# dfdazac/grapes

Hardware: AMD Instinct MI355X
Metric: sampled edges aggregated/sec, ogbn-products 3-layer GFlowNet (higher is better)
Workload: dtype f32

## Files before the change

### grapes_amd/csrc/index_kernels.hip

```cpp
#include "common.h"

__global__ void tensormap_update_k(int32_t* __restrict__ map, const int32_t* __restrict__ keys,
                                   int n_host, const int32_t* d_n) {
    const int n = eff_count(d_n, n_host);
    for (int i = blockIdx.x * blockDim.x + threadIdx.x; i < n; i += gridDim.x * blockDim.x)
        map[keys[i]] = i;
}

__global__ void tensormap_map_k(const int32_t* __restrict__ map, const int32_t* __restrict__ keys,
                                int32_t* __restrict__ out, int64_t n_host, const int32_t* d_n) {
    int64_t n = n_host;
    if (d_n) { int64_t v = *d_n; n = v < n_host ? v : n_host; }
    for (int64_t i = (int64_t)blockIdx.x * blockDim.x + threadIdx.x; i < n;
         i += (int64_t)gridDim.x * blockDim.x)
        out[i] = map[keys[i]];
}

extern "C" int grapes_tensormap_update(int32_t* map, const int32_t* keys, int32_t n,
                                       const int32_t* d_n, grapes_stream_t stream) {
    if (!map || (!keys && n > 0) || n < 0) return GRAPES_EINVAL;
    if (n == 0) return 0;
    int grid = grapes_div_up(n, 256); if (grid > 2048) grid = 2048;
    hipLaunchKernelGGL(tensormap_update_k, dim3(grid), dim3(256), 0, (hipStream_t)stream, map, keys, n, d_n);
    GRAPES_LAUNCH_CHECK();
// ... 473 lines not shown
    int grid = grapes_div_up(n, 256); if (grid > 4096) grid = 4096;
    hipLaunchKernelGGL(bitmap_mark_k, dim3(grid), dim3(256), 0, (hipStream_t)stream,
                       (unsigned long long*)bits, (unsigned long long*)bits1, ids, n, d_n, num_nodes, status);
    GRAPES_LAUNCH_CHECK();
    return 0;
}

__global__ void bitmap_mark_rows_k(unsigned long long* __restrict__ bits, unsigned long long* __restrict__ bits1,
                                   const int32_t* __restrict__ nodes, int m_host, const int32_t* d_m,
                                   const int32_t* __restrict__ eoff, int num_nodes, int32_t* status) {
    const int m = eff_count(d_m, m_host);
    for (int i = blockIdx.x * blockDim.x + threadIdx.x; i < m; i += gridDim.x * blockDim.x) {
        if (eoff[i + 1] <= eoff[i]) continue;
        const int id = nodes[i];
        if (id < 0 || id >= num_nodes) {
            if (status) atomicOr(status, GRAPES_STATUS_BAD_INDEX);
            continue;
        }
        const int w = id >> 6;
        const unsigned long long old = atomicOr(&bits[w], 1ull << (id & 63));
        if (bits1 && old == 0ull) atomicOr(&bits1[w >> 6], 1ull << (w & 63));
    }
}

extern "C" int grapes_bitmap_mark_rows(uint64_t* bits, uint64_t* bits1, const int32_t* nodes, int32_t m,
                                       const int32_t* d_m, const int32_t* eoff, int32_t num_nodes, int32_t* status,
                                       grapes_stream_t stream) {
    if (!bits || m < 0 || (m > 0 && (!nodes || !eoff))) return GRAPES_EINVAL;
    if (m == 0) return 0;
    int grid = grapes_div_up(m, 256); if (grid > 1024) grid = 1024;
    hipLaunchKernelGGL(bitmap_mark_rows_k, dim3(grid), dim3(256), 0, (hipStream_t)stream, (unsigned long long*)bits,
                       (unsigned long long*)bits1, nodes, m, d_m, eoff, num_nodes, status);
    GRAPES_LAUNCH_CHECK();
    return 0;
}

__global__ void bitmap_mark_hop_k(unsigned long long* __restrict__ prev_bits, unsigned long long* __restrict__ bits,
                                  unsigned long long* __restrict__ bits1, const int32_t* __restrict__ previous,
                                  int m_host, const int32_t* d_m, const int32_t* __restrict__ eoff,
                                  const int32_t* __restrict__ dst, int e_host, const int32_t* d_e, int num_nodes,
                                  int32_t* status) {
    const int m = eff_count(d_m, m_host);
    const int e = eff_count(d_e, e_host);
    const int stride = gridDim.x * blockDim.x;
    const int i0 = blockIdx.x * blockDim.x + threadIdx.x;
    for (int i = i0; i < m; i += stride) {
        const int id = previous[i];
        mark_bit(prev_bits, nullptr, id, num_nodes, status);
        if (eoff[i + 1] > eoff[i]) mark_bit(bits, bits1, id, num_nodes, status);
    }
    for (int t = i0; t < e; t += stride) mark_bit(bits, bits1, dst[t], num_nodes, status);
}

extern "C" int grapes_bitmap_mark_hop(uint64_t* prev_bits, uint64_t* bits, uint64_t* bits1, const int32_t* previous,
                                      int32_t m, const int32_t* d_m, const int32_t* eoff, const int32_t* dst, int32_t e,
                                      const int32_t* d_e, int32_t num_nodes, int32_t* status, grapes_stream_t stream) {
    if (!prev_bits || !bits || m < 0 || e < 0 || (m > 0 && (!previous || !eoff)) || (e > 0 && !dst))
        return GRAPES_EINVAL;
    if (m == 0 && e == 0) return 0;
    int grid = grapes_div_up(m > e ? m : e, 256); if (grid > 4096) grid = 4096;
    hipLaunchKernelGGL(bitmap_mark_hop_k, dim3(grid), dim3(256), 0, (hipStream_t)stream, (unsigned long long*)prev_bits,
                       (unsigned long long*)bits, (unsigned long long*)bits1, previous, m, d_m, eoff, dst, e, d_e, num_nodes,
                       status);
    GRAPES_LAUNCH_CHECK();
    return 0;
}

struct MarkLists { const int32_t* ids[4]; int n[4]; const int32_t* d_n[4]; };
__global__ void bitmap_mark_lists_k(unsigned long long* __restrict__ bits, unsigned long long* __restrict__ bits1,
                                    MarkLists L, int num_nodes, int32_t* status, int32_t* __restrict__ unmark_mult) {
    const int stride = gridDim.x * blockDim.x;
    const int i0 = blockIdx.x * blockDim.x + threadIdx.x;
#pragma unroll
    for (int k = 0; k < 4; ++k) {
        if (!L.ids[k]) continue;
        const int n = eff_count(L.d_n[k], L.n[k]);
        for (int i = i0; i < n; i += stride) {
            const int id = L.ids[k][i];
            mark_bit(bits, bits1, id, num_nodes, status);
            if (unmark_mult && id >= 0 && id < num_nodes) unmark_mult[id] = 0;
        }
    }
}

extern "C" int grapes_bitmap_mark_lists(uint64_t* bits, uint64_t* bits1, const int32_t* ids0, int32_t n0,
                                        const int32_t* d_n0, const int32_t* ids1, int32_t n1, const int32_t* d_n1,
                                        const int32_t* ids2, int32_t n2, const int32_t* d_n2, const int32_t* ids3,
                                        int32_t n3, const int32_t* d_n3, int32_t num_nodes, int32_t* status,
                                        int32_t* unmark_mult, grapes_stream_t stream) {
    if (!bits || n0 < 0 || n1 < 0 || n2 < 0 || n3 < 0) return GRAPES_EINVAL;
    MarkLists L{{n0 > 0 ? ids0 : nullptr, n1 > 0 ? ids1 : nullptr, n2 > 0 ? ids2 : nullptr, n3 > 0 ? ids3 : nullptr},
                {n0, n1, n2, n3}, {d_n0, d_n1, d_n2, d_n3}};
    int nmax = n0; if (n1 > nmax) nmax = n1; if (n2 > nmax) nmax = n2; if (n3 > nmax) nmax = n3;
    if (nmax == 0) return 0;
    int grid = grapes_div_up(nmax, 256); if (grid > 4096) grid = 4096;
    hipLaunchKernelGGL(bitmap_mark_lists_k, dim3(grid), dim3(256), 0, (hipStream_t)stream, (unsigned long long*)bits,
                       (unsigned long long*)bits1, L, num_nodes, status, unmark_mult);
    GRAPES_LAUNCH_CHECK();
    return 0;
}

#define UNION_MAX 4096
template <int KPT>
__device__ __forceinline__ void union_sort_regs(int* key, int tid, int P) {
    int v[KPT];
#pragma unroll
    for (int q = 0; q < KPT; ++q) v[q] = key[tid + 1024 * q];
    for (int k = 2; k <= P; k <<= 1)
        for (int j = k >> 1; j > 0; j >>= 1) {
            if (j >= 1024) {
                const int dq = j >> 10;
#pragma unroll
                for (int q = 0; q < KPT; ++q) {
                    if ((q & dq) == 0 && (q | dq) < KPT) {
                        const int q2 = q | dq;
                        const bool up = ((tid + 1024 * q) & k) == 0;
                        const int a = v[q], b = v[q2];
                        const int mn = a < b ? a : b, mx = a < b ? b : a;
                        v[q] = up ? mn : mx; v[q2] = up ? mx : mn;
                    }
                }
                continue;
            }
            int partner[KPT];
            if (j >= 64) {
                __syncthreads();
#pragma unroll
                for (int q = 0; q < KPT; ++q) key[tid + 1024 * q] = v[q];
                __syncthreads();
#pragma unroll
                for (int q = 0; q < KPT; ++q) partner[q] = key[(tid + 1024 * q) ^ j];
            } else {
#pragma unroll
                for (int q = 0; q < KPT; ++q) partner[q] = __shfl_xor(v[q], j, 64);
            }
#pragma unroll
            for (int q = 0; q < KPT; ++q) {
                const int i = tid + 1024 * q;
                const bool up = (i & k) == 0, lower = (i & j) == 0;
                const int mn = v[q] < partner[q] ? v[q] : partner[q], mx = v[q] < partner[q] ? partner[q] : v[q];
                v[q] = (lower == up) ? mn : mx;
            }
        }
    __syncthreads();
#pragma unroll
    for (int q = 0; q < KPT; ++q) key[tid + 1024 * q] = v[q];
    __syncthreads();
}
__device__ __forceinline__ void union_sorted_body(MarkLists L, int num_nodes, int n_cap, int32_t* __restrict__ out_ids,
                                                       int32_t* __restrict__ node_map, int32_t* __restrict__ counts,
                                                       int32_t* __restrict__ unmark_mult, int32_t* status) {
    __shared__ int key[UNION_MAX];
    __shared__ int lds[17];
    __shared__ int s_total;
    const int tid = threadIdx.x;
    int nh[4], cv[4], id0[4];
#pragma unroll
    for (int k = 0; k < 4; ++k) {
        nh[k] = L.ids[k] ? L.n[k] : 0;
        const int32_t* pc = (L.ids[k] && L.d_n[k]) ? L.d_n[k] : counts;
        cv[k] = *pc;
    }
#pragma unroll
    for (int k = 0; k < 4; ++k) {
        const int32_t* pi = L.ids[k] ? L.ids[k] : counts;
        id0[k] = pi[(L.ids[k] && tid < nh[k]) ? tid : 0];
    }
    int off = 0;
    bool bad = false;
#pragma unroll
    for (int k = 0; k < 4; ++k) {
        if (!L.ids[k]) continue;
        int n = nh[k];
        if (L.d_n[k]) { n = cv[k] < nh[k] ? (cv[k] < 0 ? 0 : cv[k]) : nh[k]; }
        for (int i = tid; i < n; i += blockDim.x) {
            const int id = i == tid ? id0[k] : L.ids[k][i];
            const bool ok = id >= 0 && id < num_nodes;
            bad = bad || !ok;
            key[off + i] = ok ? id : 0x7fffffff;
        }
        off += n;
    }
    int P = 1; while (P < off) P <<= 1;
    for (int i = off + tid; i < P; i += blockDim.x) key[i] = 0x7fffffff;
    if (bad && status) atomicOr(status, GRAPES_STATUS_BAD_INDEX);
    __syncthreads();
    if (P <= (int)blockDim.x) {
        int v = tid < P ? key[tid] : 0x7fffffff;
        for (int k = 2; k <= P; k <<= 1)
            for (int j = k >> 1; j > 0; j >>= 1) {
                int partner;
                if (j >= 64) {
                    __syncthreads();
                    key[tid] = v;
                    __syncthreads();
                    partner = key[tid ^ j];
                } else {
                    partner = __shfl_xor(v, j, 64);
                }
                const bool up = (tid & k) == 0, lower = (tid & j) == 0;
                const int mn = v < partner ? v : partner, mx = v < partner ? partner : v;
                v = (lower == up) ? mn : mx;
            }
        __syncthreads();
        key[tid] = v;
        __syncthreads();
    } else if (blockDim.x == 1024 && (P == 2048 || P == 4096)) {
        if (P == 2048) union_sort_regs<2>(key, tid, P); else union_sort_regs<4>(key, tid, P);
    } else
    for (int k = 2; k <= P; k <<= 1)
        for (int j = k >> 1; j > 0; j >>= 1) {
            for (int i = tid; i < P; i += blockDim.x) {
                const int ixj = i ^ j;
                if (ixj > i) {
                    const int a = key[i], b = key[ixj];
                    const bool up = (i & k) == 0;
                    if ((a > b) == up) { key[i] = b; key[ixj] = a; }
                }
            }
            __syncthreads();
        }
    const int per = (P + (int)blockDim.x - 1) / (int)blockDim.x;
    const int lo = tid * per, hi = lo + per < P ? lo + per : P;
    int mine = 0;
    for (int i = lo; i < hi; ++i) { const int v = key[i]; if (v != 0x7fffffff && (i == 0 || key[i - 1] != v)) ++mine; }
    int tot;
    int pos = block_excl_scan(mine, lds, &tot);
    bool overflow = false;
    for (int i = lo; i < hi; ++i) {
        const int v = key[i];
        if (v != 0x7fffffff && (i == 0 || key[i - 1] != v)) {
            if (pos < n_cap) { out_ids[pos] = v; if (node_map) node_map[v] = pos; }
            else overflow = true;
            if (unmark_mult) unmark_mult[v] = 0;
            ++pos;
        }
    }
    if (tid == 0) { counts[0] = tot < n_cap ? tot : n_cap; counts[1] = counts[0]; }
    if (overflow && status) atomicOr(status, GRAPES_STATUS_NODE_OVERFLOW);
    (void)s_total;
}

__global__ __launch_bounds__(1024) void union_sorted_k(MarkLists L, int num_nodes, int n_cap, int32_t* __restrict__ out_ids,
                                                       int32_t* __restrict__ node_map, int32_t* __restrict__ counts,
                                                       int32_t* __restrict__ unmark_mult, int32_t* status) {
    union_sorted_body(L, num_nodes, n_cap, out_ids, node_map, counts, unmark_mult, status);
}

extern "C" int grapes_bitmap_clear(uint64_t* bits, const int32_t* ids, int64_t n, const int32_t* d_n,
                                   grapes_stream_t stream) {
    if (!bits || (!ids && n > 0) || n < 0) return GRAPES_EINVAL;
    if (n == 0) return 0;
    int grid = grapes_div_up(n, 256); if (grid > 4096) grid = 4096;
    hipLaunchKernelGGL(bitmap_clear_k, dim3(grid), dim3(256), 0, (hipStream_t)stream,
                       (unsigned long long*)bits, ids, n, d_n);
    GRAPES_LAUNCH_CHECK();
    return 0;
}

__global__ __launch_bounds__(1024) void compact_count_k(const unsigned long long* __restrict__ bits,
                                                        const unsigned long long* __restrict__ prev_bits, int W,
                                                        int32_t* __restrict__ bsum_b, int32_t* __restrict__ bsum_n) {
    __shared__ int lds[17];
    const int q = blockIdx.x * blockDim.x + threadIdx.x;
    int cb = 0, cn = 0;
    if (q < W) {
        const unsigned long long bb = bits[q];
        if (bb) {
            const unsigned long long pp = prev_bits ? prev_bits[q] : 0ull;
            cb = __popcll(bb); cn = __popcll(bb & ~pp);
        }
    }
    int tb, tn;
    block_excl_scan(cb, lds, &tb);
    block_excl_scan(cn, lds, &tn);
    if (threadIdx.x == 0) { bsum_b[blockIdx.x] = tb; bsum_n[blockIdx.x] = tn; }
}

__device__ __forceinline__ void long_row_items(const grapes_hop_degree_args& hd, int row, int ct, int cs) {
    if (ct > GRAPES_LONG_ROW) {
        const int nc = (ct + GRAPES_LONG_ROW - 1) / GRAPES_LONG_ROW;
        const int b0 = atomicAdd(&hd.n_long[0], nc);
        for (int c = 0; c < nc; ++c)
            if (b0 + c < hd.item_cap) { hd.long_items[2 * (b0 + c)] = row; hd.long_items[2 * (b0 + c) + 1] = c; }
    }
    if (cs > GRAPES_LONG_ROW) {
        const int nc = (cs + GRAPES_LONG_ROW - 1) / GRAPES_LONG_ROW;
        const int b0 = atomicAdd(&hd.n_long[1], nc);
        for (int c = 0; c < nc; ++c)
            if (b0 + c < hd.item_cap) { hd.long_items[2 * (hd.item_cap + b0 + c)] = row; hd.long_items[2 * (hd.item_cap + b0 + c) + 1] = c; }
    }
}

__device__ __forceinline__ void compact_emit_body(unsigned long long* __restrict__ bits,
                                                       const unsigned long long* __restrict__ prev_bits, int W,
                                                       const int32_t* __restrict__ bsum_b, const int32_t* __restrict__ bsum_n,
                                                       int n_cap, int32_t* __restrict__ batch_nodes,
                                                       int32_t* __restrict__ neighbor_nodes, int32_t* __restrict__ nb_local,
                                                       int32_t* __restrict__ node_map, int32_t* __restrict__ counts,
                                                       int32_t* status, uint32_t* __restrict__ ind_code,
                                                       uint32_t epoch_host, const uint32_t* d_epoch, int ind_bit,
                                                       unsigned long long* __restrict__ sync, int32_t* __restrict__ cand_pos,
                                                       uint32_t* __restrict__ zero_a, size_t words_a,
                                                       uint32_t* __restrict__ zero_b, size_t words_b,
                                                       uint32_t* __restrict__ zero_c, size_t words_c,
                                                       grapes_slice_remark_args rm, int gc,
                                                       grapes_hop_degree_args hd, const int BID, const int NBLK) {
    const int sj_t = blockDim.x > 64 ? (int)blockDim.x - 64 : (int)blockDim.x, sj_0 = blockDim.x > 64 ? (int)threadIdx.x - 64 : (int)threadIdx.x;
    if (BID >= gc) {
        if (sj_0 < 0) return;
        const size_t stride = (size_t)NBLK * sj_t, i0 = (size_t)BID * sj_t + sj_0;
        if (rm.mult) {
            if (rm.unmark_ids) { const int c = eff_count(rm.d_n_unmark, rm.n_unmark); for (size_t i = i0; i < (size_t)c; i += stride) rm.mult[rm.unmark_ids[i]] = 0; }
            if (rm.mark_ids) { const int c = eff_count(rm.d_n_mark, rm.n_mark); for (size_t i = i0; i < (size_t)c; i += stride) atomicAdd(&rm.mult[rm.mark_ids[i]], 1); }
        }
        for (size_t i = i0; i < words_a; i += stride) zero_a[i] = 0u;
        for (size_t i = i0; i < words_b; i += stride) zero_b[i] = 0u;
        for (size_t i = i0; i < words_c; i += stride) zero_c[i] = 0u;
        return;
    }
    __shared__ int lds[51];
    __shared__ unsigned long long lds64[2];
    GRAPES_STAMP_NW(0);
    const uint32_t epoch = d_epoch ? (*d_epoch & 0xffffffu) : epoch_host;
    const int w = BID * blockDim.x + threadIdx.x;
    unsigned long long bb = 0ull, pp = 0ull;
    int wt = 0, wsv = 0;
    if (w < W) {
        bb = bits[w];
        pp = prev_bits ? prev_bits[w] : 0ull;
        if (hd.indeg) { wt = hd.wsum[w]; wsv = hd.wsum[W + w]; }
    }
    GRAPES_STAMP(1);
    int tb, tn;
    int posb, posn;
    int post = 0, poss = 0, tt = 0, ts = 0;
    if (blockDim.x <= 512 && hd.indeg) {
        int pk = __popcll(bb) | (__popcll(bb & ~pp) << 16), tot;
        post = wt; poss = wsv;
        block_excl_scan3(pk, post, poss, lds, &tot, &tt, &ts);
        posb = pk & 0xffff; posn = (int)((unsigned)pk >> 16); tb = tot & 0xffff; tn = (int)((unsigned)tot >> 16);
    } else if (blockDim.x <= 512) {
        int tot;
        const int pk = block_excl_scan(__popcll(bb) | (__popcll(bb & ~pp) << 16), lds, &tot);
        posb = pk & 0xffff; posn = (int)((unsigned)pk >> 16); tb = tot & 0xffff; tn = (int)((unsigned)tot >> 16);
    } else {
        posb = block_excl_scan(__popcll(bb), lds, &tb);
        posn = block_excl_scan(__popcll(bb & ~pp), lds, &tn);
    }
    GRAPES_STAMP_NW(7);
    if (sync && threadIdx.x == 0)
        __hip_atomic_store(&sync[1 + BID], (1ull << 63) | ((unsigned long long)tn << 31) | (unsigned)tb, __ATOMIC_RELAXED, __HIP_MEMORY_SCOPE_AGENT);
    constexpr int PRE = 4;
    int l_ct[PRE] = {0, 0, 0, 0}, l_lp[PRE] = {0, 0, 0, 0};
    uint32_t l_cd[PRE] = {0u, 0u, 0u, 0u};
    int2 l_sg[PRE] = {make_int2(0, 0), make_int2(0, 0), make_int2(0, 0), make_int2(0, 0)};
    if (hd.indeg) {
        if (blockDim.x > 512) {
            post = block_excl_scan(wt, lds, &tt);
            poss = block_excl_scan(wsv, lds, &ts);
        }
        if (sync && threadIdx.x == 0)
            __hip_atomic_store(&((unsigned long long*)hd.sync2)[1 + BID], (1ull << 63) | ((unsigned long long)(unsigned)ts << 31) | (unsigned)tt, __ATOMIC_RELAXED, __HIP_MEMORY_SCOPE_AGENT);
        GRAPES_STAMP_NW(8);
        if (sync) { unsigned long long dummy2; (void)lookback_exclusive2(sync, (unsigned long long*)hd.sync2, BID, lds64, status, &dummy2, 1); }
        const uint32_t* icp = ind_code ? ind_code : reinterpret_cast<const uint32_t*>(hd.indeg);
        unsigned long long b2 = bb;
#pragma unroll
        for (int k = 0; k < PRE; ++k) {
            const bool has = b2 != 0ull;
            const int b = has ? __ffsll((long long)b2) - 1 : 0;
            b2 &= b2 - 1;
            const bool isprev = has && ((pp >> b) & 1ull) != 0ull;
            const int id = has ? w * 64 + b : 0, idp = isprev ? id : 0, idn = (has && !isprev) ? id : 0;
            l_ct[k] = hd.indeg[id];
            l_sg[k] = *reinterpret_cast<const int2*>(hd.seginfo + 2 * (long long)idp);
            l_lp[k] = hd.loops[idp];
            l_cd[k] = icp[idn];
        }
        if (w < W) { if (wt) hd.wsum[w] = 0; if (wsv) hd.wsum[W + w] = 0; }
    }
    GRAPES_STAMP_NW(2);
    if (w < W && bb) bits[w] = 0ull;
    if (rm.mult && sj_0 >= 0) {
        const int stride = NBLK * sj_t, i0 = BID * sj_t + sj_0;
        if (rm.unmark_ids) { const int c = eff_count(rm.d_n_unmark, rm.n_unmark); for (int i = i0; i < c; i += stride) rm.mult[rm.unmark_ids[i]] = 0; }
        if (rm.mark_ids) { const int c = eff_count(rm.d_n_mark, rm.n_mark); for (int i = i0; i < c; i += stride) atomicAdd(&rm.mult[rm.mark_ids[i]], 1); }
    }
    if (sj_0 >= 0) {
        const size_t stride = (size_t)NBLK * sj_t, i0 = (size_t)BID * sj_t + sj_0;
        for (size_t i = i0; i < words_a; i += stride) zero_a[i] = 0u;
        for (size_t i = i0; i < words_b; i += stride) zero_b[i] = 0u;
        for (size_t i = i0; i < words_c; i += stride) zero_c[i] = 0u;
// ... 933 lines not shown
```

### grapes_amd/csrc/loss_kernels.hip

```cpp
#include "common.h"
#include "row_loss.h"

#define LOSS_THREADS 1024
#define LOSS_MAX_B 4096

__device__ __forceinline__ float block_sum_fixed(const float* v, int n, float* red) {
    float acc = 0.f;
    for (int i = threadIdx.x; i < n; i += blockDim.x) acc += v[i];
    acc = wave_sum(acc);
    __syncthreads();
    if (lane_id() == 0) red[threadIdx.x >> 6] = acc;
    __syncthreads();
    float t = 0.f;
    for (int w = 0; w < (int)(blockDim.x >> 6); ++w) t += red[w];
    return t;
}

__device__ __forceinline__ void gflownet_loss_eval(bool has_z, float log_z_raw, float log_z_init,
                                                   const float* __restrict__ stats, int hops, int stride, float cost,
                                                   float loss_coef, int reinforce, float* __restrict__ out) {
    float tot = stats[4];
    for (int h = 1; h < hops; ++h) tot = __fadd_rn(tot, stats[h * stride + 4]);
    const float lz = has_z ? __fsub_rn(log_z_raw, log_z_init) : 0.f;
    float loss, scale;
    if (reinforce) {
        loss = __fmul_rn(-tot, cost);
        scale = -cost;
    } else {
        const float inner = __fadd_rn(__fadd_rn(lz, tot), __fmul_rn(loss_coef, cost));
        loss = __fmul_rn(inner, inner);
        scale = __fmul_rn(2.0f, inner);
    }
    out[0] = loss; out[1] = scale; out[2] = lz; out[3] = tot;
}

struct GfnTail {
    float* out4;
    const float* zout; int nz; const int32_t* d_nz; float log_z_init;
    const float* stats; int hops, stride; float loss_coef; int reinforce;
    const float* loss_extra;
};

__device__ __forceinline__ float loss_row(const float* __restrict__ logits, float* __restrict__ dlogits, int n_rows, int C,
                                          int row, long long gid, const int64_t* __restrict__ labels,
                                          const float* __restrict__ labels_f, int multilabel, float inv, int lane) {
    float loss = 0.f;
    if ((unsigned)row < (unsigned)n_rows) {
        const RowStrided r{logits + (long long)row * C, dlogits + (long long)row * C, C, lane};
        loss = multilabel ? row_loss_bce(r, labels_f + gid * C, inv)
                          : row_loss_ce<CE_LOG_SOFTMAX>(r, (int)labels[gid], inv);
    }
    return loss;
}

__global__ __launch_bounds__(LOSS_THREADS) void classifier_loss_k(
    const float* __restrict__ logits, int n_rows, int C, const int32_t* __restrict__ local_rows,
    const int32_t* __restrict__ node_map ,
    const int32_t* __restrict__ target_ids, const int64_t* __restrict__ labels, const float* __restrict__ labels_f,
    int B, int multilabel, float* __restrict__ dlogits, float* __restrict__ loss_out, GfnTail gt) {
    __shared__ float row_loss[LOSS_MAX_B];
    __shared__ float red[LOSS_THREADS / 64];
    __shared__ double zred[LOSS_THREADS / 64];
    const int tid = threadIdx.x, lane = lane_id(), wid = tid >> 6, nw = blockDim.x >> 6;
    const long long total = (long long)n_rows * C;
    double zs = 0.0;
    int nzv = 0;
    if (gt.out4 && gt.zout) {
        nzv = eff_count(gt.d_nz, gt.nz);
        for (int i = tid; i < nzv; i += blockDim.x) zs += (double)gt.zout[i];
    }
    if ((((uintptr_t)dlogits) & 15) == 0) {
        float4* d4 = reinterpret_cast<float4*>(dlogits);
        const long long n4 = total >> 2;
        for (long long i = tid; i < n4; i += blockDim.x) d4[i] = make_float4(0.f, 0.f, 0.f, 0.f);
        for (long long i = (n4 << 2) + tid; i < total; i += blockDim.x) dlogits[i] = 0.f;
    } else {
        for (long long i = tid; i < total; i += blockDim.x) dlogits[i] = 0.f;
    }
    __syncthreads();
    const float inv = multilabel ? 1.0f / ((float)B * (float)C) : 1.0f / (float)B;
    if (!multilabel && C <= 64) {
        constexpr int RIF = 16;
        for (int b0 = wid * RIF; b0 < B; b0 += nw * RIF) {
            int row[RIF]; long long gid[RIF];
#pragma unroll
            for (int u = 0; u < RIF; ++u) {
                const int b = b0 + u < B ? b0 + u : B - 1;
                gid[u] = target_ids[b];
                row[u] = local_rows ? local_rows[b] : node_map[gid[u]];
            }
            float xv[RIF]; int yv[RIF];
#pragma unroll
            for (int u = 0; u < RIF; ++u) {
                const bool ok = (unsigned)row[u] < (unsigned)n_rows;
                const int r = ok ? row[u] : 0;
                xv[u] = logits[(long long)r * C + (lane < C ? lane : 0)];
                yv[u] = (int)labels[gid[u]];
            }
#pragma unroll
            for (int u = 0; u < RIF; ++u) {
                if (b0 + u >= B) continue;
                const bool ok = (unsigned)row[u] < (unsigned)n_rows;
                const float x = lane < C ? xv[u] : -INFINITY;
                const float m = wave_max(x);
                const float se = wave_sum(lane < C ? expf(x - m) : 0.f);
                const float lsm = (x - m) - logf(se);
                const float l = wave_sum((lane == yv[u] && lane < C) ? -lsm : 0.f);
                if (ok && lane < C) dlogits[(long long)row[u] * C + lane] = (expf(lsm) - (lane == yv[u] ? 1.0f : 0.0f)) * inv;
                if (lane == 0) row_loss[b0 + u] = ok ? l : 0.f;
            }
        }
    } else
    for (int b = wid; b < B; b += nw) {
        const long long gid = target_ids[b];
        const int row = local_rows ? local_rows[b] : node_map[gid];
        const float loss = loss_row(logits, dlogits, n_rows, C, row, gid, labels, labels_f, multilabel, inv, lane);
        if (lane == 0) row_loss[b] = loss;
    }
    __syncthreads();
    const float s = block_sum_fixed(row_loss, B, red);
    const float lc = s * inv + (gt.loss_extra ? *gt.loss_extra : 0.f);
    if (tid == 0) *loss_out = lc;
    if (!gt.out4) return;
    zs = wave_sum_d(zs);
    if (lane == 0) zred[wid] = zs;
    __syncthreads();
    if (tid == 0) {
        double t = 0.0;
        for (int w = 0; w < nw; ++w) t += zred[w];
        const float zmean = (float)(nzv > 0 ? t / (double)nzv : 0.0 / 0.0);
        gflownet_loss_eval(gt.zout != nullptr, zmean, gt.log_z_init, gt.stats, gt.hops, gt.stride, lc, gt.loss_coef,
                           gt.reinforce, gt.out4);
    }
}

#define LOSS_MB_THREADS 256
#define LOSS_MB_MAXROWS 65536
__global__ __launch_bounds__(LOSS_MB_THREADS) void step_losses_mb_k(
    const float* __restrict__ logits, int n_rows, int C, const int32_t* __restrict__ node_map,
    const int32_t* __restrict__ target_ids, const int64_t* __restrict__ labels, const float* __restrict__ labels_f,
    int B, int multilabel, float* __restrict__ dlogits, float* __restrict__ loss_out, GfnTail gt,
    float* __restrict__ row_loss , unsigned* __restrict__ ticket) {
    __shared__ unsigned bm[LOSS_MB_MAXROWS / 32];
    __shared__ double dred[16];
    __shared__ float fred[16];
    __shared__ int s_last;
    const int tid = threadIdx.x, lane = lane_id(), wid = tid >> 6;
    const int G = gridDim.x;
    double* zslot = reinterpret_cast<double*>(row_loss + ((B + 1) & ~1));
    const float inv = multilabel ? 1.0f / ((float)B * (float)C) : 1.0f / (float)B;
    if (blockIdx.x == 0) {
        if (gt.out4 && gt.zout) {
            const int nz = eff_count(gt.d_nz, gt.nz);
            double zs[4] = {0.0, 0.0, 0.0, 0.0};
            for (int i0 = 0; i0 < nz; i0 += 8 * 1024) {
                float xv[8][4];
#pragma unroll
                for (int u = 0; u < 8; ++u)
#pragma unroll
                    for (int q = 0; q < 4; ++q) {
                        const int i = i0 + 1024 * u + tid + 256 * q;
                        xv[u][q] = gt.zout[i < nz ? i : nz - 1];
                    }
#pragma unroll
                for (int u = 0; u < 8; ++u)
#pragma unroll
                    for (int q = 0; q < 4; ++q) { if (i0 + 1024 * u + tid + 256 * q < nz) zs[q] += (double)xv[u][q]; }
            }
#pragma unroll
            for (int q = 0; q < 4; ++q) { const double w = wave_sum_d(zs[q]); if (lane == 0) dred[wid + 4 * q] = w; }
            __syncthreads();
            if (tid == 0) {
                double t = 0.0;
                for (int w = 0; w < 16; ++w) t += dred[w];
                publish_f64(zslot, t);
            }
        }
    } else {
        const int nwords = (n_rows + 31) >> 5;
        const int nwv = (G - 1) * (blockDim.x >> 6);
        const int b_first = (blockIdx.x - 1) * (blockDim.x >> 6) + wid;
        const long long gid_first = target_ids[b_first < B ? b_first : 0];
        const int tb = tid < B ? tid : 0;
        const long long gid_t = target_ids[tb];
        const int row_first = node_map[gid_first];
        const int row_t = node_map[gid_t];
        for (int i = tid; i < nwords; i += blockDim.x) bm[i] = 0u;
        __syncthreads();
        for (int b = tid; b < B; b += blockDim.x) {
            const int row = b == tid ? row_t : node_map[target_ids[b]];
            if ((unsigned)row < (unsigned)n_rows) atomicOr(&bm[row >> 5], 1u << (row & 31));
        }
        __syncthreads();
        const long long total = (long long)n_rows * C;
        const long long n4 = ((((uintptr_t)dlogits) & 15) == 0) ? (total >> 2) : 0;
        const long long stride = (long long)(G - 1) * blockDim.x;
        for (long long i = (long long)(blockIdx.x - 1) * blockDim.x + tid; i < n4; i += stride) {
            const int r0 = (int)((4 * i) / C), r1 = (int)((4 * i + 3) / C);
            const bool t0 = (bm[r0 >> 5] >> (r0 & 31)) & 1u, t1 = (bm[r1 >> 5] >> (r1 & 31)) & 1u;
            if (!t0 && !t1) {
                reinterpret_cast<float4*>(dlogits)[i] = make_float4(0.f, 0.f, 0.f, 0.f);
            } else {
#pragma unroll
                for (int u = 0; u < 4; ++u) { const int r = (int)((4 * i + u) / C); if (!((bm[r >> 5] >> (r & 31)) & 1u)) dlogits[4 * i + u] = 0.f; }
            }
        }
        for (long long i = (n4 << 2) + (long long)(blockIdx.x - 1) * blockDim.x + tid; i < total; i += stride) {
            const int r = (int)(i / C);
            if (!((bm[r >> 5] >> (r & 31)) & 1u)) dlogits[i] = 0.f;
        }
        for (int b = b_first; b < B; b += nwv) {
            const long long gid = b == b_first ? gid_first : (long long)target_ids[b];
            const int row = b == b_first ? row_first : node_map[gid];
            const float l = loss_row(logits, dlogits, n_rows, C, row, gid, labels, labels_f, multilabel, inv, lane);
            if (lane == 0) publish_f32(&row_loss[b], l);
        }
    }
    __syncthreads();
    if (tid == 0) s_last = (atomicAdd(ticket, 1u) == (unsigned)G - 1) ? 1 : 0;
    __syncthreads();
    if (!s_last) return;
    float ls[4] = {0.f, 0.f, 0.f, 0.f};
    for (int i0 = 0; i0 < B; i0 += 1024) {
#pragma unroll
        for (int q = 0; q < 4; ++q) {
            const int i = i0 + tid + 256 * q;
            if (i < B) ls[q] += __int_as_float(__hip_atomic_load((const int*)(row_loss + i), __ATOMIC_RELAXED, __HIP_MEMORY_SCOPE_AGENT));
        }
    }
#pragma unroll
    for (int q = 0; q < 4; ++q) { const float w = wave_sum(ls[q]); if (lane == 0) fred[wid + 4 * q] = w; }
    __syncthreads();
    if (tid == 0) {
        float t = 0.f;
        for (int w = 0; w < 16; ++w) t += fred[w];
        const float loss = t * inv + (gt.loss_extra ? *gt.loss_extra : 0.f);
        *loss_out = loss;
        *ticket = 0u;
        if (gt.out4) {
            float zmean = 0.f;
            if (gt.zout) {
                const int nz = eff_count(gt.d_nz, gt.nz);
                const double zt = __longlong_as_double(__hip_atomic_load((const long long*)zslot, __ATOMIC_RELAXED, __HIP_MEMORY_SCOPE_AGENT));
                zmean = (float)(nz > 0 ? zt / (double)nz : 0.0 / 0.0);
            }
            gflownet_loss_eval(gt.zout != nullptr, zmean, gt.log_z_init, gt.stats, gt.hops, gt.stride, loss, gt.loss_coef,
                               gt.reinforce, gt.out4);
        }
    }
}

__global__ void gflownet_loss_k(const float* __restrict__ log_z_raw, float log_z_init, const float* __restrict__ stats,
                                int hops, int stride, const float* __restrict__ loss_c, float loss_coef, int reinforce,
                                float* __restrict__ out ) {
    if (threadIdx.x != 0 || blockIdx.x != 0) return;
    gflownet_loss_eval(log_z_raw != nullptr, log_z_raw ? *log_z_raw : 0.f, log_z_init, stats, hops, stride, *loss_c,
                       loss_coef, reinforce, out);
}

struct AdamTensor {
    float* p; const float* g; float* m; float* v; float* step;
    long long n;
    double lr, beta1, beta2, eps, weight_decay;
    int maximize; int pad_;
    float* w_pad; void* img; int K; int ld_pad;
};
typedef __bf16 adam_bf16;
__device__ __forceinline__ void adam_mirror(const AdamTensor& d, long long i, float pnew) {
    const unsigned iu = (unsigned)i, Ku = (unsigned)d.K;
    const int nrow = (int)(iu / Ku), k = (int)(iu - (unsigned)nrow * Ku);
    if (d.w_pad) d.w_pad[(long long)nrow * d.ld_pad + k] = pnew;
    if (d.img) {
        const adam_bf16 h = (adam_bf16)pnew;
        const float r1 = pnew - (float)h;
        const adam_bf16 m = (adam_bf16)r1;
        const adam_bf16 l = (adam_bf16)(r1 - (float)m);
        adam_bf16* o = reinterpret_cast<adam_bf16*>(d.img) +
                       ((((long long)(k >> 5) * 3 * 4 + ((k >> 3) & 3)) * GRAPES_TS_IMG_ROWS + nrow) * 8 + (k & 7));
        o[0] = h; o[(long long)4 * GRAPES_TS_IMG_ROWS * 8] = m; o[(long long)8 * GRAPES_TS_IMG_ROWS * 8] = l;
    }
}

#define ADAM_MAX_SETS 8
struct AdamSlabs { int nsets; int k_host; const int32_t* d_k; int accumulate; const float* slabs[ADAM_MAX_SETS]; const float* out[ADAM_MAX_SETS]; };
__device__ __forceinline__ float adam_slab_combine8(const float (&v)[8], int ns) {
    const int per = (ns + 3) >> 2;
    float part[4];
#pragma unroll
    for (int g = 0; g < 4; ++g) {
        const int z0 = g * per, z1 = (z0 + per < ns) ? z0 + per : ns;
        float acc = 0.f;
#pragma unroll
        for (int z = 0; z < 8; ++z) acc = (z >= z0 && z < z1) ? acc + v[z] : acc;
        part[g] = acc;
    }
    return (part[0] + part[1]) + (part[2] + part[3]);
}
__device__ __forceinline__ float adam_slab_sum(const float* __restrict__ sl, long long cnt, long long i, int ns) {
    if (ns <= 0) return 0.f;
    const int per = (ns + 3) >> 2;
    float part[4];
    if (ns <= 8) {
        float v[8];
#pragma unroll
        for (int z = 0; z < 8; ++z) v[z] = sl[(long long)(z < ns ? z : ns - 1) * cnt + i];
        return adam_slab_combine8(v, ns);
    }
#pragma unroll
    for (int g = 0; g < 4; ++g) {
        const int z0 = g * per, z1 = (z0 + per < ns) ? z0 + per : ns;
        float acc = 0.f;
        for (int z = z0; z < z1; ++z) acc += sl[(long long)z * cnt + i];
        part[g] = acc;
    }
    return (part[0] + part[1]) + (part[2] + part[3]);
}
__global__ __launch_bounds__(256) void adam_step_k(const AdamTensor* __restrict__ desc, int n_tensors,
                                                   unsigned* __restrict__ ticket, AdamSlabs sb) {
    __shared__ int s_last;
    const AdamTensor d = desc[blockIdx.y];
    const float* sl = nullptr;
#pragma unroll
    for (int q = 0; q < ADAM_MAX_SETS; ++q) if (q < sb.nsets && sb.out[q] == d.g) sl = sb.slabs[q];
    const int ns = sl ? (eff_count(sb.d_k, sb.k_host) + DWS_ROWS - 1) / DWS_ROWS : 0;
    const float stepv = *d.step;
    const long long stride = (long long)gridDim.x * blockDim.x;
    const long long i0 = (long long)blockIdx.x * blockDim.x + threadIdx.x;
    const float omb1 = (float)(1.0 - d.beta1), b2 = (float)d.beta2, omb2 = (float)(1.0 - d.beta2);
    const float eps = (float)d.eps, wd = (float)d.weight_decay;
    float step_size = 0.f, bc2_sqrt = 1.f;
    bool have = false;
    for (long long base = i0; base < d.n; base += 4 * stride) {
        float g[4], p[4], m[4], v[4];
#pragma unroll
        for (int u = 0; u < 4; ++u) {
            const long long i = base + u * stride;
            const long long ic = i < d.n ? i : base;
            typedef const __attribute__((address_space(1))) float* gcf;
            g[u] = ((gcf)d.g)[ic]; p[u] = ((gcf)d.p)[ic]; m[u] = ((gcf)d.m)[ic]; v[u] = ((gcf)d.v)[ic];
        }
        const bool gzero = sl && !sb.accumulate;
        if (sl && ns > 0 && ns <= 8) {
            float sv[4][8];
#pragma unroll
            for (int u = 0; u < 4; ++u) {
                const long long i = base + u * stride;
                const long long ic = i < d.n ? i : base;
#pragma unroll
                for (int z = 0; z < 8; ++z) sv[u][z] = sl[(long long)(z < ns ? z : ns - 1) * d.n + ic];
            }
#pragma unroll
            for (int u = 0; u < 4; ++u) {
                const long long i = base + u * stride;
                const float t = adam_slab_combine8(sv[u], ns);
                g[u] = sb.accumulate ? g[u] + t : t;
                if (i < d.n) const_cast<float*>(d.g)[i] = g[u];
            }
        } else if (sl) {
#pragma unroll
            for (int u = 0; u < 4; ++u) {
                const long long i = base + u * stride;
                if (gzero) g[u] = 0.f;
                if (i < d.n) {
                    const float t = adam_slab_sum(sl, d.n, i, ns);
                    g[u] = sb.accumulate ? g[u] + t : t;
                    const_cast<float*>(d.g)[i] = g[u];
                }
            }
        }
        if (!have) {
            const float fs = (float)((double)stepv + 1.0);
            const double bc1 = 1.0 - (double)exp2f(fs * log2f((float)d.beta1));
            const double bc2 = 1.0 - (double)exp2f(fs * log2f((float)d.beta2));
            step_size = (float)(d.lr / bc1);
            bc2_sqrt = (float)sqrt(bc2);
            have = true;
        }
#pragma unroll
        for (int u = 0; u < 4; ++u) {
            const long long i = base + u * stride;
            if (i < d.n) {
                float gg = d.maximize ? -g[u] : g[u];
                if (wd != 0.f) gg = __fmaf_rn(wd, p[u], gg);
                const float mm = m[u] + (gg - m[u]) * omb1;
                const float vv = b2 * v[u] + omb2 * (gg * gg);
                const float denom = sqrtf(vv) / bc2_sqrt + eps;
                const float pnew = p[u] - step_size * (mm / denom);
                d.p[i] = pnew;
                d.m[i] = mm; d.v[i] = vv;
                if (d.w_pad || d.img) adam_mirror(d, i, pnew);
            }
        }
    }
    __syncthreads();
    if (threadIdx.x == 0) {
        const unsigned t = atomicAdd(&ticket[blockIdx.y], 1u);
        s_last = (t == gridDim.x - 1) ? 1 : 0;
    }
    __syncthreads();
    if (s_last && threadIdx.x == 0) {
// ... 269 lines not shown
```

Baseline: 506.9 million.

## Prefetch loads early in union sort and loss kernels to hide latency

```diff
diff --git a/grapes_amd/csrc/index_kernels.hip b/grapes_amd/csrc/index_kernels.hip
--- a/grapes_amd/csrc/index_kernels.hip
+++ b/grapes_amd/csrc/index_kernels.hip
@@ -649,28 +649,35 @@
                                                        int32_t* __restrict__ unmark_mult, int32_t* status) {
     __shared__ int key[UNION_MAX];
     __shared__ int lds[17];
-    __shared__ int s_total;
     const int tid = threadIdx.x;
+    const int T = __builtin_amdgcn_readfirstlane((int)blockDim.x);
     int nh[4], cv[4], id0[4];
+    int zoff = 0;
+    asm volatile("" : "+v"(zoff));
 #pragma unroll
     for (int k = 0; k < 4; ++k) {
         nh[k] = L.ids[k] ? L.n[k] : 0;
+        const int32_t* pi = L.ids[k] ? L.ids[k] : counts;
+        id0[k] = pi[zoff + ((L.ids[k] && tid < nh[k]) ? tid : 0)];
+    }
+#pragma unroll
+    for (int k = 0; k < 4; ++k) {
         const int32_t* pc = (L.ids[k] && L.d_n[k]) ? L.d_n[k] : counts;
-        cv[k] = *pc;
+        cv[k] = pc[zoff];
     }
 #pragma unroll
     for (int k = 0; k < 4; ++k) {
-        const int32_t* pi = L.ids[k] ? L.ids[k] : counts;
-        id0[k] = pi[(L.ids[k] && tid < nh[k]) ? tid : 0];
-    }
+        const int c = __builtin_amdgcn_readfirstlane(cv[k]);
+        cv[k] = (L.ids[k] && L.d_n[k]) ? (c < nh[k] ? (c < 0 ? 0 : c) : nh[k]) : nh[k];
+    }
+    asm volatile("" :: "v"(id0[0]), "v"(id0[1]), "v"(id0[2]), "v"(id0[3]));
     int off = 0;
     bool bad = false;
 #pragma unroll
     for (int k = 0; k < 4; ++k) {
         if (!L.ids[k]) continue;
-        int n = nh[k];
-        if (L.d_n[k]) { n = cv[k] < nh[k] ? (cv[k] < 0 ? 0 : cv[k]) : nh[k]; }
-        for (int i = tid; i < n; i += blockDim.x) {
+        const int n = cv[k];
+        for (int i = tid; i < n; i += T) {
             const int id = i == tid ? id0[k] : L.ids[k][i];
             const bool ok = id >= 0 && id < num_nodes;
             bad = bad || !ok;
@@ -679,10 +686,10 @@
         off += n;
     }
     int P = 1; while (P < off) P <<= 1;
-    for (int i = off + tid; i < P; i += blockDim.x) key[i] = 0x7fffffff;
+    for (int i = off + tid; i < P; i += T) key[i] = 0x7fffffff;
     if (bad && status) atomicOr(status, GRAPES_STATUS_BAD_INDEX);
     __syncthreads();
-    if (P <= (int)blockDim.x) {
+    if (P <= T) {
         int v = tid < P ? key[tid] : 0x7fffffff;
         for (int k = 2; k <= P; k <<= 1)
             for (int j = k >> 1; j > 0; j >>= 1) {
@@ -702,12 +709,12 @@
         __syncthreads();
         key[tid] = v;
         __syncthreads();
-    } else if (blockDim.x == 1024 && (P == 2048 || P == 4096)) {
+    } else if (T == 1024 && (P == 2048 || P == 4096)) {
         if (P == 2048) union_sort_regs<2>(key, tid, P); else union_sort_regs<4>(key, tid, P);
     } else
     for (int k = 2; k <= P; k <<= 1)
         for (int j = k >> 1; j > 0; j >>= 1) {
-            for (int i = tid; i < P; i += blockDim.x) {
+            for (int i = tid; i < P; i += T) {
                 const int ixj = i ^ j;
                 if (ixj > i) {
                     const int a = key[i], b = key[ixj];
@@ -717,7 +724,7 @@
             }
             __syncthreads();
         }
-    const int per = (P + (int)blockDim.x - 1) / (int)blockDim.x;
+    const int per = (P + T - 1) / T;
     const int lo = tid * per, hi = lo + per < P ? lo + per : P;
     int mine = 0;
     for (int i = lo; i < hi; ++i) { const int v = key[i]; if (v != 0x7fffffff && (i == 0 || key[i - 1] != v)) ++mine; }
@@ -735,7 +742,6 @@
     }
     if (tid == 0) { counts[0] = tot < n_cap ? tot : n_cap; counts[1] = counts[0]; }
     if (overflow && status) atomicOr(status, GRAPES_STATUS_NODE_OVERFLOW);
-    (void)s_total;
 }
 
 __global__ __launch_bounds__(1024) void union_sorted_k(MarkLists L, int num_nodes, int n_cap, int32_t* __restrict__ out_ids,
diff --git a/grapes_amd/csrc/loss_kernels.hip b/grapes_amd/csrc/loss_kernels.hip
--- a/grapes_amd/csrc/loss_kernels.hip
+++ b/grapes_amd/csrc/loss_kernels.hip
@@ -16,11 +16,8 @@
     return t;
 }
 
-__device__ __forceinline__ void gflownet_loss_eval(bool has_z, float log_z_raw, float log_z_init,
-                                                   const float* __restrict__ stats, int hops, int stride, float cost,
-                                                   float loss_coef, int reinforce, float* __restrict__ out) {
-    float tot = stats[4];
-    for (int h = 1; h < hops; ++h) tot = __fadd_rn(tot, stats[h * stride + 4]);
+__device__ __forceinline__ void gflownet_loss_finish(bool has_z, float log_z_raw, float log_z_init, float tot, float cost,
+                                                     float loss_coef, int reinforce, float* __restrict__ out) {
     const float lz = has_z ? __fsub_rn(log_z_raw, log_z_init) : 0.f;
     float loss, scale;
     if (reinforce) {
@@ -32,6 +29,13 @@
         scale = __fmul_rn(2.0f, inner);
     }
     out[0] = loss; out[1] = scale; out[2] = lz; out[3] = tot;
+}
+__device__ __forceinline__ void gflownet_loss_eval(bool has_z, float log_z_raw, float log_z_init,
+                                                   const float* __restrict__ stats, int hops, int stride, float cost,
+                                                   float loss_coef, int reinforce, float* __restrict__ out) {
+    float tot = stats[4];
+    for (int h = 1; h < hops; ++h) tot = __fadd_rn(tot, stats[h * stride + 4]);
+    gflownet_loss_finish(has_z, log_z_raw, log_z_init, tot, cost, loss_coef, reinforce, out);
 }
 
 struct GfnTail {
@@ -136,6 +140,13 @@
 
 #define LOSS_MB_THREADS 256
 #define LOSS_MB_MAXROWS 65536
+#define LOSS_MB_PRE_HOPS 4
+struct RowHeld {
+    float xv; float* __restrict__ g; int C, lane;
+    template <class F> __device__ __forceinline__ void each(F f) const { if (lane < C) f(0, lane); }
+    __device__ __forceinline__ float get(int, int) const { return xv; }
+    __device__ __forceinline__ void put(int, int c, float v) const { g[c] = v; }
+};
 __global__ __launch_bounds__(LOSS_MB_THREADS) void step_losses_mb_k(
     const float* __restrict__ logits, int n_rows, int C, const int32_t* __restrict__ node_map,
     const int32_t* __restrict__ target_ids, const int64_t* __restrict__ labels, const float* __restrict__ labels_f,
@@ -149,9 +160,19 @@
     const int G = gridDim.x;
     double* zslot = reinterpret_cast<double*>(row_loss + ((B + 1) & ~1));
     const float inv = multilabel ? 1.0f / ((float)B * (float)C) : 1.0f / (float)B;
+    int zoff = 0;
+    asm volatile("" : "+v"(zoff));
+    const float* anyw = reinterpret_cast<const float*>(zslot);
+    const bool has4 = gt.out4 != nullptr;
+    const float pre_extra = (gt.loss_extra ? gt.loss_extra : anyw)[zoff];
+    const int pre_dnz = reinterpret_cast<const int32_t*>(gt.d_nz ? reinterpret_cast<const float*>(gt.d_nz) : anyw)[zoff];
+    float pre_st[LOSS_MB_PRE_HOPS];
+#pragma unroll
+    for (int h = 0; h < LOSS_MB_PRE_HOPS; ++h)
+        pre_st[h] = (has4 ? gt.stats : anyw)[zoff + ((has4 && h < gt.hops) ? h * gt.stride + 4 : 0)];
     if (blockIdx.x == 0) {
         if (gt.out4 && gt.zout) {
-            const int nz = eff_count(gt.d_nz, gt.nz);
+            const int nz = __builtin_amdgcn_readfirstlane(gt.d_nz ? (pre_dnz < gt.nz ? (pre_dnz < 0 ? 0 : pre_dnz) : gt.nz) : gt.nz);
             double zs[4] = {0.0, 0.0, 0.0, 0.0};
             for (int i0 = 0; i0 < nz; i0 += 8 * 1024) {
                 float xv[8][4];
@@ -179,19 +200,28 @@
     } else {
         const int nwords = (n_rows + 31) >> 5;
         const int nwv = (G - 1) * (blockDim.x >> 6);
-        const int b_first = (blockIdx.x - 1) * (blockDim.x >> 6) + wid;
+        const int b_first = (blockIdx.x - 1) * (blockDim.x >> 6) + wid, b_second = b_first + nwv;
+        const bool held = !multilabel && C <= 64;
         const long long gid_first = target_ids[b_first < B ? b_first : 0];
+        const long long gid_second = target_ids[b_second < B ? b_second : 0];
         const int tb = tid < B ? tid : 0;
         const long long gid_t = target_ids[tb];
         const int row_first = node_map[gid_first];
+        const int row_second = node_map[gid_second];
         const int row_t = node_map[gid_t];
+        const int64_t* lp = held ? labels : reinterpret_cast<const int64_t*>(zslot);
+        const int y_first = (int)lp[held ? gid_first : 0], y_second = (int)lp[held ? gid_second : 0];
+        const bool ok_first = (unsigned)row_first < (unsigned)n_rows, ok_second = (unsigned)row_second < (unsigned)n_rows;
+        const int cl = (held && lane < C) ? lane : 0;
+        const float x_first = logits[(long long)(ok_first ? row_first : 0) * C + cl];
+        const float x_second = logits[(long long)(ok_second ? row_second : 0) * C + cl];
         for (int i = tid; i < nwords; i += blockDim.x) bm[i] = 0u;
-        __syncthreads();
+        lds_barrier();
         for (int b = tid; b < B; b += blockDim.x) {
             const int row = b == tid ? row_t : node_map[target_ids[b]];
             if ((unsigned)row < (unsigned)n_rows) atomicOr(&bm[row >> 5], 1u << (row & 31));
         }
-        __syncthreads();
+        lds_barrier();
         const long long total = (long long)n_rows * C;
         const long long n4 = ((((uintptr_t)dlogits) & 15) == 0) ? (total >> 2) : 0;
         const long long stride = (long long)(G - 1) * blockDim.x;
@@ -209,24 +239,40 @@
             const int r = (int)(i / C);
             if (!((bm[r >> 5] >> (r & 31)) & 1u)) dlogits[i] = 0.f;
         }
-        for (int b = b_first; b < B; b += nwv) {
+        int b_next = b_first;
+        if (held) {
+            float l_first = 0.f, l_second = 0.f;
+            if (b_first < B && ok_first)
+                l_first = row_loss_ce<CE_LOG_SOFTMAX>(RowHeld{x_first, dlogits + (long long)row_first * C, C, lane}, y_first, inv);
+            if (b_second < B && ok_second)
+                l_second = row_loss_ce<CE_LOG_SOFTMAX>(RowHeld{x_second, dlogits + (long long)row_second * C, C, lane}, y_second, inv);
+            if (lane < 2 && (lane ? b_second : b_first) < B)
+                publish_f32(&row_loss[lane ? b_second : b_first], lane ? l_second : l_first);
+            b_next = b_second + nwv;
+        }
+        for (int b = b_next; b < B; b += nwv) {
             const long long gid = b == b_first ? gid_first : (long long)target_ids[b];
             const int row = b == b_first ? row_first : node_map[gid];
             const float l = loss_row(logits, dlogits, n_rows, C, row, gid, labels, labels_f, multilabel, inv, lane);
             if (lane == 0) publish_f32(&row_loss[b], l);
         }
     }
+    asm volatile("" :: "v"(pre_extra), "v"(pre_dnz), "v"(pre_st[0]), "v"(pre_st[1]), "v"(pre_st[2]), "v"(pre_st[3]));
     __syncthreads();
     if (tid == 0) s_last = (atomicAdd(ticket, 1u) == (unsigned)G - 1) ? 1 : 0;
     __syncthreads();
     if (!s_last) return;
+    const double zt = __longlong_as_double(__hip_atomic_load((const long long*)zslot, __ATOMIC_RELAXED, __HIP_MEMORY_SCOPE_AGENT));
     float ls[4] = {0.f, 0.f, 0.f, 0.f};
     for (int i0 = 0; i0 < B; i0 += 1024) {
+        float rv[4];
 #pragma unroll
         for (int q = 0; q < 4; ++q) {
             const int i = i0 + tid + 256 * q;
-            if (i < B) ls[q] += __int_as_float(__hip_atomic_load((const int*)(row_loss + i), __ATOMIC_RELAXED, __HIP_MEMORY_SCOPE_AGENT));
-        }
+            rv[q] = __int_as_float(__hip_atomic_load((const int*)(row_loss + (i < B ? i : 0)), __ATOMIC_RELAXED, __HIP_MEMORY_SCOPE_AGENT));
+        }
+#pragma unroll
+        for (int q = 0; q < 4; ++q) { if (i0 + tid + 256 * q < B) ls[q] += rv[q]; }
     }
 #pragma unroll
     for (int q = 0; q < 4; ++q) { const float w = wave_sum(ls[q]); if (lane == 0) fred[wid + 4 * q] = w; }
@@ -234,18 +280,20 @@
     if (tid == 0) {
         float t = 0.f;
         for (int w = 0; w < 16; ++w) t += fred[w];
-        const float loss = t * inv + (gt.loss_extra ? *gt.loss_extra : 0.f);
+        const float loss = t * inv + (gt.loss_extra ? pre_extra : 0.f);
         *loss_out = loss;
         *ticket = 0u;
         if (gt.out4) {
             float zmean = 0.f;
             if (gt.zout) {
-                const int nz = eff_count(gt.d_nz, gt.nz);
-                const double zt = __longlong_as_double(__hip_atomic_load((const long long*)zslot, __ATOMIC_RELAXED, __HIP_MEMORY_SCOPE_AGENT));
+                const int nz = gt.d_nz ? (pre_dnz < gt.nz ? (pre_dnz < 0 ? 0 : pre_dnz) : gt.nz) : gt.nz;
                 zmean = (float)(nz > 0 ? zt / (double)nz : 0.0 / 0.0);
             }
-            gflownet_loss_eval(gt.zout != nullptr, zmean, gt.log_z_init, gt.stats, gt.hops, gt.stride, loss, gt.loss_coef,
-                               gt.reinforce, gt.out4);
+            float tot = pre_st[0];
+#pragma unroll
+            for (int h = 1; h < LOSS_MB_PRE_HOPS; ++h) { if (h < gt.hops) tot = __fadd_rn(tot, pre_st[h]); }
+            for (int h = LOSS_MB_PRE_HOPS; h < gt.hops; ++h) tot = __fadd_rn(tot, gt.stats[h * gt.stride + 4]);
+            gflownet_loss_finish(gt.zout != nullptr, zmean, gt.log_z_init, tot, loss, gt.loss_coef, gt.reinforce, gt.out4);
         }
     }
 }
```

New measurement: 511.0 million, median of 6. No clear change (+0.8%).
